# achao2013/deep3dmap

Measured on AMD Instinct MI355X. Metric: rendered Mpix/s fwd+bwd, 100k-tri mesh @512x512, higher is better.
Workload: dtype f32

## Files before the change

deep3dmap_amd/_lib.py:

```python
import ctypes
import os

import torch

from .build import LOAD_PATH as LIB_PATH

_c_f32p = ctypes.c_void_p
_I, _F, _SZ, _L = ctypes.c_int, ctypes.c_float, ctypes.c_size_t, ctypes.c_long
_P = ctypes.c_void_p


class D3MCamera(ctypes.Structure):
    _fields_ = [("mode", _I), ("perspective", _I), ("tan_half_width", _F), ("orig_size", _F),
                ("rot", _P), ("eye_or_t", _P), ("K", _P), ("dist", _P),
                ("rot_batch", _I), ("eye_batch", _I), ("K_batch", _I), ("dist_batch", _I)]


class D3MBasis(ctypes.Structure):
    _fields_ = [("eye", _P), ("at_or_direction", _P), ("up", _P), ("eye_batch", _I), ("at_batch", _I), ("up_batch", _I),
                ("is_look_at", _I)]


class D3MCameraGrad(ctypes.Structure):
    _fields_ = [("eye_or_t", _P), ("at_or_direction", _P), ("up", _P), ("rot", _P), ("K", _P), ("dist", _P)]
# ... 8 lines not shown
    _fields_ = [("intensity_ambient", _P), ("intensity_directional", _P), ("color_ambient", _P), ("color_directional", _P),
                ("direction", _P), ("ia_batch", _I), ("id_batch", _I), ("ca_batch", _I), ("cd_batch", _I), ("dir_batch", _I)]


class D3MMeshTopology(ctypes.Structure):
    _fields_ = ([(n, _P) for n in ("nbr_offsets", "nbr_items", "wings", "wing_offsets", "wing_items", "nbr_chunks",
                                   "nbr_long_rows", "nbr_long_chunk_ptr", "wing_chunks", "wing_long_rows",
                                   "wing_long_chunk_ptr")] +
                [(n, _I) for n in ("num_vertices", "num_edges", "num_wings", "num_nbr_chunks", "num_nbr_long_rows",
                                   "num_wing_chunks", "num_wing_long_rows", "long_row")])


class D3MFitTargets(ctypes.Structure):
    _fields_ = [("rgb_target", _P), ("depth_target", _P), ("alpha_target", _P), ("mask", _P), ("scratch", _P),
                ("loss", _P), ("grad_rgb_map", _P), ("grad_alpha_map", _P), ("grad_depth_map", _P), ("grad_loss", _P),
                ("mask_sum", _P), ("edge_grad", _P), ("edge_dot", _P), ("edge_nz_lo_inv", _P), ("edge_nz_hi1", _P), ("flags", _I)]


class D3MG2SBlock(ctypes.Structure):
    _fields_ = ([("batch_size", _I), ("height", _I), ("width", _I), ("image_size", _I), ("anti_aliasing", _I), ("flip", _I),
                 ("inv_K", _P), ("inv_K_batch", _I), ("K", _P), ("K_batch", _I),
                 ("rot_center_depth", _F), ("depth_min", _F), ("depth_max", _F), ("near", _F), ("far", _F),
                 ("camera", ctypes.POINTER(D3MCamera)), ("view", _P), ("view_components", _I)] +
                [(n, _P) for n in ("rot", "trans", "depth", "albedo", "light_a", "light_b", "light_d", "target", "extra_mask",
                                   "normal", "diffuse_shading", "texture", "recon_depth", "recon_im", "recon_im_mask",
                                   "losses")] +
                [("lam_smooth", _F), ("with_smooth", _I)] +
                [(n, _P) for n in ("screen_vertices", "zbuffer", "scratch",
                                   "grad_recon_im", "grad_l1", "grad_l1_flip", "grad_smooth", "grad_total",
                                   "grad_texture", "grad_tri", "grad_depth_map", "grad_normal", "grad_depth_mesh",
                                   "grad_depth", "grad_albedo", "grad_light_a", "grad_light_b", "grad_light_d", "grad_rot",
# ... 70 lines not shown
    "d3m_face_light": (_I, [_P, _I, _P, _I, _P, _F, _F, _P, _P, _P, _I, _I, _I, _I, _P]),
    "d3m_face_light_backward": (_I, [_P, _I, _P, _I, _P, _P, _F, _F, _P, _P, _P, _I, _I, _I, _I, _P]),
    "d3m_face_light_dev": (_I, [_P, _I, _P, _I, _P, ctypes.POINTER(D3MLight), _I, _I, _I, _I, _P]),
    "d3m_face_light_backward_dev": (_I, [_P, _I, _P, _I, _P, _P, ctypes.POINTER(D3MLight), _I, _I, _I, _I, _P]),
    "d3m_face_light_backward_gather_dev": (_I, [_P, _P, _P, _P, _P, _P, ctypes.POINTER(D3MLight), _I, _I, _I, _P]),
    "d3m_light_params_backward_workspace_bytes": (_SZ, [_I, _I, _I]),
    "d3m_light_params_backward": (_I, [_P, _I, _P, _I, _P, _I, ctypes.POINTER(D3MLight), ctypes.POINTER(D3MLight), _I, _I, _I,
                                       _P, _SZ, _P]),
    "d3m_forward_texture_sampling_lit": (_I, [_P, _P, _I, _P, _I, _P, _P, _P, _P, _I, _I, _I, _I, _I, _F, _P]),
    "d3m_backward_textures_lit_workspace_bytes": (_SZ, [_I, _I, _I, _I]),
    "d3m_render_lit_epilogue": (_I, [_P, _P, _I, _P, _I, _P, _P, _P, _P, _I, _P, _P, _P, _P, _P, _I, _I, _I, _I, _I, _F, _I,
                                     _P, _P]),
    "d3m_render_fit_scratch_floats": (_SZ, [_I, _I]),
    "d3m_render_fit_scratch_clear_range": (_SZ, [_I, _I, ctypes.POINTER(_SZ)]),
    "d3m_fit_finish": (_I, [ctypes.POINTER(D3MFitTargets), _I, _I, _P]),
    "d3m_fit_loss_records": (_I, [_P, _P, _P, _P, ctypes.POINTER(D3MFitTargets), _I, _I, _P]),
    "d3m_backward_textures_lit": (_I, [_P, _P, _I, _P, _I, _P, _P, _P, _P, _P, _P, _P, _P, _I, _I, _I, _I, _I, _F, _P, _SZ,
                                       _P, _P, _P, _I, _P]),
    "d3m_backward_textures_lit_clear_ranges": (_I, [_P, _I, _P, _I, _I, _I, _I, _I, _P, _I, ctypes.POINTER(_P),
                                                    ctypes.POINTER(_SZ)]),
    "d3m_lit_back": (_I, [_P, _I, ctypes.POINTER(D3MCamera), _P, _P, _I, _I, _P, _I, _I, _I, _P, _I, _F, _F, _P, _P, _P, _P]),
    "d3m_lit_back_dev": (_I, [_P, _I, ctypes.POINTER(D3MCamera), _P, _P, _I, _I, _P, _I, _I, _I, _P, _I, ctypes.POINTER(D3MLight),
                              _P]),
    "d3m_lit_front_dev": (_I, [_P, _I, ctypes.POINTER(D3MCamera), ctypes.POINTER(D3MBasis), _P, _I, _I, _P, _I, _I, _I, _P, _I,
                               ctypes.POINTER(D3MLight), ctypes.POINTER(_P), ctypes.POINTER(_SZ), _I, _P]),
    "d3m_lit_front": (_I, [_P, _I, ctypes.POINTER(D3MCamera), ctypes.POINTER(D3MBasis), _P, _I, _I, _P, _I, _I, _I, _P, _I,
                           _F, _F, _P, _P, _P, ctypes.POINTER(_P), ctypes.POINTER(_SZ), _I, _P]),
    "d3m_output_epilogue": (_I, [_P, _P, _P, _P, _I, _P, _P, _P, _P, _P, _I, _I, _I, _P]),
    "d3m_output_epilogue_backward": (_I, [_P, _P, _P, _P, _P, _P, _I, _I, _I, _P]),
    "d3m_output_epilogue_backward_records": (_I, [_P, _P, _P, _P, _P, _P, _P, _P, _P, _P, _P, _I, _I, _I, _P]),
# ... 172 lines not shown
```

deep3dmap_amd/csrc/d3m_edge_grad.h:

```cpp
#pragma once
#include <algorithm>
#include <atomic>
#include <type_traits>
#include "d3m_backward.h"
#include "d3m_face_major.h"
#include "d3m_launch.h"

namespace d3m {

#ifndef D3M_EG_INLINE_MAX
#define D3M_EG_INLINE_MAX 6
#endif
constexpr int EG_INLINE_MAX = D3M_EG_INLINE_MAX;
#ifndef D3M_EG_LINE_WAVES
#define D3M_EG_LINE_WAVES 8
#endif
constexpr int EG_LINE_WAVES = D3M_EG_LINE_WAVES;
constexpr int EG_ITEM_DW = 8;

struct EdgeGradArgs {
    const float4* grad;
    const float2* dot;
    const float* go;
    __device__ __forceinline__ size_t pixel(int axis, size_t view_base, int d0, int d1) const {
// ... 15 lines not shown
    int img_s, img_aa;
    __device__ __forceinline__ bool direct() const { return ga_map != nullptr || ga_img != nullptr; }
    __device__ __forceinline__ float direct_ga(size_t pi) const {
        if (ga_map) return ga_map[pi];
        const size_t plane = (size_t)S * S;
        const int b = (int)(pi / plane), rem = (int)(pi - (size_t)b * plane), y = rem / S, x = rem - y * S;
        const int yo = img_aa ? (S - 1 - y) >> 1 : S - 1 - y, xo = img_aa ? x >> 1 : x;
        return ga_img[((size_t)b * img_s + yo) * img_s + xo] * (img_aa ? 0.25f : 1.0f);
    }
    __device__ __forceinline__ float direct_ga_at(size_t view, int axis, int d0, int d1, size_t pi) const {
        if (ga_map) return ga_map[pi];
        const int y = axis ? d0 : d1, x = axis ? d1 : d0;
        const int yo = img_aa ? (S - 1 - y) >> 1 : S - 1 - y, xo = img_aa ? x >> 1 : x;
        return ga_img[(view * img_s + yo) * img_s + xo] * (img_aa ? 0.25f : 1.0f);
    }
    __device__ __forceinline__ float4 rec_grad(size_t pi) const {
        return direct() ? make_float4(direct_ga(pi), 0.0f, 0.0f, 0.0f) : grad[pi];
    }
    __device__ __forceinline__ float2 rec_dot(size_t pi) const {
        if (!direct()) return dot[pi];
        return make_float2(alpha_map[pi] * direct_ga(pi), __int_as_float(fi_direct[pi]));
    }
    __device__ __forceinline__ int extent_lo(size_t line) const { return nz_lo_inv ? S - nz_lo_inv[line] : 0; }
    __device__ __forceinline__ int extent_hi(size_t line) const { return nz_hi1 ? nz_hi1[line] - 1 : S - 1; }
    int* line_left;
    int* n_left;
};

struct SegRef {
    float alpha, r, g, b;
};

struct Segment {
    int axis, d0, from, to, inward, f0, f1;
// ... 133 lines not shown
__device__ __forceinline__ void visit_pixel_div(float diff, int d1, float d1_cross, float q0, float q1, bool f0, bool f1,
                                                float two_over_is, float eps, float& g0, float& g1) {
    const float t = (float)d1 - d1_cross;
    float dist0 = q0 * t * two_over_is;
    dist0 = (0 < dist0) ? dist0 + eps : dist0 - eps;
    float dist1 = q1 * t * two_over_is;
    dist1 = (0 < dist1) ? dist1 + eps : dist1 - eps;
    const bool skip = diff <= 0;
    g0 -= (skip || !f0) ? 0.0f : diff / dist0;
    g1 -= (skip || !f1) ? 0.0f : diff / dist1;
}

__device__ __forceinline__ SegRef load_ref(const EdgeGradArgs& a, int axis, size_t view_base, int d0, int d1) {
    const size_t idx = view_base + (axis ? (size_t)d0 * a.S + d1 : (size_t)d1 * a.S + d0);
    SegRef r = {0, 0, 0, 0};
    if (a.use_alpha) r.alpha = a.alpha_map[idx];
    if (a.use_rgb) { r.r = a.rgb_map[3 * idx + 0]; r.g = a.rgb_map[3 * idx + 1]; r.b = a.rgb_map[3 * idx + 2]; }
    return r;
}

__device__ __forceinline__ void inline_pixel(const Segment& sg, const SegRef& ref, int fn, const float2 dt, const float4 g,
                                             int d1, bool on, float two_over_is, float eps, float& g0, float& g1) {
    float diff = dt.x;
    diff = __builtin_fmaf(-ref.alpha, g.x, diff);
    diff = __builtin_fmaf(-ref.r, g.y, diff);
    diff = __builtin_fmaf(-ref.g, g.z, diff);
    diff = __builtin_fmaf(-ref.b, g.w, diff);
    if (!on || (sg.inward && __float_as_int(dt.y) != fn)) diff = 0.0f;
    visit_pixel(diff, d1, sg.d1_cross, sg.f0 ? sg.q0 : 1.0f, sg.f1 ? sg.q1 : 1.0f, sg.f0 != 0, sg.f1 != 0, two_over_is, eps,
                g0, g1);
// ... 592 lines not shown
    const size_t view_base = bn * is * is;
    const int x_first = __builtin_amdgcn_readfirstlane(line_first_record(w, line));
    const uint4* xrec = w.xrec + (size_t)x_first;
    const float two_over_is = 2.0f / (float)is;
    const int p_lo = __builtin_amdgcn_readfirstlane(a.extent_lo(line));
    const int p_hi = __builtin_amdgcn_readfirstlane(a.extent_hi(line));
    auto load_record = [&](int ci) {
        uint4 r = make_uint4(0, 0, 0, 0);
        if (ci < n_x) r = xrec[(uint32_t)ci];
        return r;
    };
    float2* s_df = (float2*)s_line;
    float4* s_grd = (float4*)(s_df + is + (is & 1));
    float4* s_val = s_grd + is;
    const float go_sign = a.go_sign();
    for (int p = (int)threadIdx.x; p < is; p += EG_LINE_THREADS) {
        const size_t pi = a.pixel(axis, view_base, d0, p);
        float4 v = make_float4(0, 0, 0, 0);
        if (USE_ALPHA) v.x = a.alpha_map[pi];
        if (USE_RGB) { v.y = a.rgb_map[3 * pi]; v.z = a.rgb_map[3 * pi + 1]; v.w = a.rgb_map[3 * pi + 2]; }
        s_val[p] = v;
    }
    for (int p = p_lo + (int)threadIdx.x; p <= p_hi; p += EG_LINE_THREADS) {
        const size_t pi = a.pixel(axis, view_base, d0, p);
        float4 g;
        float2 d;
        if (!USE_RGB && a.direct()) {
            const float ga = a.direct_ga_at(bn, axis, d0, p, pi);
            g = make_float4(ga, 0.0f, 0.0f, 0.0f);
            d = make_float2(a.alpha_map[pi] * ga, __int_as_float(a.fi_direct[pi]));
        } else {
            g = a.grad[pi];
            d = a.dot[pi];
        }
        g.x *= go_sign; g.y *= go_sign; g.z *= go_sign; g.w *= go_sign;
        s_grd[p] = g;
        s_df[p] = make_float2(0.5f * go_sign * d.x, d.y);
    }
    typedef float v2f __attribute__((ext_vector_type(2)));
    auto diff_of = [](const float4 g, const float2 d, const v2f nref_ar, const v2f nref_gb) {
        v2f p = {d.x, d.x};
        p = __builtin_elementwise_fma(v2f{g.x, g.y}, nref_ar, p);
// ... 754 lines not shown
}

inline size_t edge_grad_workspace_min_bytes(int B, int F, int S) {
    return edge_layout(B, F, S).fixed_bytes + edge_plan_min_bytes(B, F, S);
}
inline size_t edge_grad_workspace_bytes(int B, int F, int S) {
    return edge_layout(B, F, S).fixed_bytes + edge_plan_bytes(B, F, S);
}

struct EdgeRecords {
    const float4* grad;
    const float2* dot;
    const int* nz_lo_inv;
    const int* nz_hi1;
    const float* go;
    const float* ga_img = nullptr;
    int img_aa = 0;
};

inline size_t edge_lines_lds(int S) {
    const size_t pairs = (size_t)(S + (S & 1)) * 8, body = pairs + (size_t)S * 32;
    return std::max(body, pairs + (size_t)(2 * S + 32) * 16);
}

template <class FS>
int run_edge_grad(FS fs, PixelMaps m, float* grad_faces, VertexTarget vt, const VisibilityView* shared_vis,
                  void* shared_plan, size_t shared_plan_bytes, EdgeRecords rec, GradScale gs, int B, float eps, void* ws,
                  size_t ws_bytes, hipStream_t st, int* last_err) {
    const int S = m.S, F = fs.num_faces();
    if (S > 65535 || F > (1 << 25) || (long)B * 2 * S >= (1l << 31)) return 1;
// ... 15 lines not shown
    EdgePlan w;
    if (shared_plan) {
        if (!edge_plan_view(shared_plan, shared_plan_bytes, vis, B, F, S, w)) return 2;
    } else {
        if (!edge_plan_view(p + L.off_plan, ws_bytes - L.fixed_bytes, vis, B, F, S, w)) return 2;
        e = run_edge_plan(fs, m.face_index_map, w, p + L.off_plan, B, S, st);
        if (e != hipSuccess) { *last_err = (int)e; return 3; }
    }
    float4* grad_row = (float4*)(p + L.off_grad_row);
    float2* dot_row = (float2*)(p + L.off_dot_row);
    float2* lane_partial = (float2*)(p + L.off_lane_partial);
    EdgeGradArgs a;
    a.ga_map = a.ga_img = nullptr; a.fi_direct = m.face_index_map; a.img_s = S; a.img_aa = 0;
    const bool direct = !rec.grad && !m.use_rgb && m.use_alpha && !gs.totals &&
                        (rec.ga_img || d3m_env_int("D3M_EG_DIRECT", 1) != 0);
    if (rec.grad) {
        a.grad = rec.grad; a.dot = rec.dot; a.go = rec.go;
        a.nz_lo_inv = rec.nz_lo_inv; a.nz_hi1 = rec.nz_hi1;
    } else if (direct) {
        a.grad = nullptr; a.dot = nullptr; a.go = nullptr; a.nz_lo_inv = a.nz_hi1 = nullptr;
        if (rec.ga_img) { a.ga_img = rec.ga_img; a.img_aa = rec.img_aa; a.img_s = rec.img_aa ? S / 2 : S; }
        else a.ga_map = m.grad_alpha_map;
    } else {
        e = zero_async(p + L.off_nz_lo, L.nz_bytes, st);
        if (e != hipSuccess) { *last_err = (int)e; return 3; }
        LAUNCH("k_pack_maps", k_pack_maps, dim3((S + 31) / 32, (S + 31) / 32, B), dim3(256), st, m.face_index_map,
               m.use_alpha ? m.alpha_map : nullptr, m.use_alpha ? m.grad_alpha_map : nullptr,
               m.use_rgb ? m.rgb_map : nullptr, m.use_rgb ? m.grad_rgb_map : nullptr, grad_row, dot_row,
               (int*)(p + L.off_nz_lo), (int*)(p + L.off_nz_hi), S, gs);
        a.grad = grad_row; a.dot = dot_row; a.go = nullptr;
        a.nz_lo_inv = (const int*)(p + L.off_nz_lo); a.nz_hi1 = (const int*)(p + L.off_nz_hi);
    }
    a.alpha_map = m.alpha_map; a.rgb_map = m.rgb_map;
// ... 48 lines not shown
```

deep3dmap_amd/csrc/d3m_lit.h:

```cpp
#pragma once
#include "d3m_aux.h"
#include "d3m_tail.h"
#include "d3m_face_major.h"

namespace d3m {

struct LitTextures {
    const float* textures;
    const float* light;
    int F, Fp, ts, tex_batch, light_batch, fill_back;
    const float* im;
    int im_H, im_W;
};

__device__ __forceinline__ long lit_texel(const LitTextures& t, int B, int b, int fp, int isc, int* light_row) {
    const int ts3 = t.ts * t.ts * t.ts;
    long vf = (long)b * t.Fp + fp + isc / ts3;
    isc %= ts3;
    if (vf >= (long)B * t.Fp) return -1;
    const int bb = (int)(vf / t.Fp), ff = (int)(vf % t.Fp);
    *light_row = (t.light_batch > 1 ? bb : 0) * t.Fp + ff;
    int fo = ff, idx = isc;
    if (ff >= t.F) {
        fo = ff - t.F;
// ... 413 lines not shown
    }
}

template <int TILE>
__device__ __forceinline__ unsigned tile_row_mask(unsigned long long ball) {
    const int sub = (int)(threadIdx.x & 63) / TILE;
    return (unsigned)(ball >> (sub * TILE)) & (TILE == 32 ? 0xFFFFFFFFu : (1u << (TILE & 31)) - 1u);
}
struct FitRecords {
    float4* grad;
    float2* dot;
    int* nz_lo_inv;
    int* nz_hi1;
    const float* mask_sum;
    float* g_depth;
};

#ifndef D3M_FIT_MINWAVES
#define D3M_FIT_MINWAVES 4
#endif
template <int TILE>
__global__ void __launch_bounds__(256, D3M_FIT_MINWAVES) k_render_lit_fit_records(const float* __restrict__ faces, LitTextures lt,
                                                               const int32_t* __restrict__ face_index_map,
                                                               const float* __restrict__ weight_map,
                                                               const float* __restrict__ depth_map,
                                                               const float* __restrict__ background, int bg_b,
                                                               float* __restrict__ rgb_blended, float* __restrict__ alpha_map,
                                                               float* __restrict__ rgb_out, float* __restrict__ alpha_out,
                                                               float* __restrict__ depth_out,
                                                               int B, int S, float eps, FitTargets fit, FitRecords rec) {
    static_assert(TILE == 32 || TILE == 16, "tile of 32 x 32 or 16 x 16 pixels");
    constexpr int ROWS = 256 / TILE;
    __shared__ float4 s_part[4];
    __shared__ int s_col_lo_inv[TILE], s_col_hi1[TILE];
    if (threadIdx.x < TILE) { s_col_lo_inv[threadIdx.x] = 0; s_col_hi1[threadIdx.x] = 0; }
    __syncthreads();
    const int b = blockIdx.z, x0 = blockIdx.x * TILE, y0 = blockIdx.y * TILE;
    const int tx = threadIdx.x % TILE, ty = threadIdx.x / TILE;
    const float* bg = background + (size_t)(bg_b > 1 ? b : 0) * 3;
    const float inv_pixels = 1.0f / (float)((long)S * S), inv_3den = 1.0f / (3.0f * *rec.mask_sum);
    float t_rgb = 0, t_d = 0, t_m = 0, t_sse = 0;
    auto sgn = [](float x) { return x > 0 ? 1.0f : (x < 0 ? -1.0f : 0.0f); };
    for (int r = ty; r < TILE; r += ROWS) {
        const int yi = y0 + r, xi = x0 + tx;
        bool nz = false;
        if (yi < S && xi < S) {
            const int yo = S - 1 - yi;
            const size_t p = ((size_t)b * S + yi) * S + xi, o = ((size_t)b * S + yo) * S + xi;
            float tg[6];
#pragma unroll
            for (int k = 0; k < 3; k++) tg[k] = fit.rgb_t[(((size_t)b * 3 + k) * S + yo) * S + xi];
            tg[3] = fit.depth_t[o]; tg[4] = fit.alpha_t[o]; tg[5] = fit.mask[o];
            const int fi = face_index_map[p];
            const float depth = depth_map[p];
            float v[3] = {bg[0], bg[1], bg[2]};
            if (fi >= 0) {
                const float weight[3] = {weight_map[3 * p], weight_map[3 * p + 1], weight_map[3 * p + 2]};
                sample_pixel_lit(faces, lt, B, b, fi, weight, depth, eps, v);
            }
            const float alpha = fi >= 0 ? 1.0f : 0.0f;
#pragma unroll
            for (int k = 0; k < 3; k++) rgb_blended[3 * p + k] = v[k];
            alpha_map[p] = alpha;
            if (rgb_out) {
#pragma unroll
                for (int k = 0; k < 3; k++) rgb_out[(((size_t)b * 3 + k) * S + yo) * S + xi] = v[k];
            }
// ... 747 lines not shown
```

deep3dmap_amd/csrc/d3m_raster.hip:

```cpp
#include <hip/hip_runtime.h>
#include <stdint.h>
#include <stdio.h>
#include <string.h>

#include "../../include/d3m_raster.h"
#include "d3m_launch.h"
#include "d3m_aux.h"
#include "d3m_textures.h"
#include "d3m_vertex_colors.h"
#include "d3m_mesh_reg.h"
#include "d3m_morphable.h"
#include "d3m_pose.h"
#include "d3m_mesh.h"
#include "d3m_uv.h"
#include "d3m_backward.h"
#include "d3m_device.h"
#include "d3m_edge_grad.h"
#include "d3m_face_major.h"
#include "d3m_forward.h"
#include "d3m_lit.h"
#include "d3m_g2s.h"
#include "d3m_bid.h"
#include "d3m_front.h"
#include "d3m_light_grad.h"
// ... 426 lines not shown
        num_faces <= 0 || image_size <= 0 || texture_size <= 0)
        return D3M_ERR_INVALID;
    const long n = (long)batch_size * image_size * image_size;
    LAUNCH("k_texture_sampling", k_texture_sampling, dim3(blocks_for(n, 256)), dim3(256), (hipStream_t)stream, faces, textures,
                       face_index_map, weight_map, depth_map, rgb_map, sampling_index_map, sampling_weight_map,
                       batch_size, num_faces, image_size, texture_size, eps);
    return check_launch();
}

static GradScale to_grad_scale(const d3m_fit_targets* unscaled, int image_size) {
    if (!unscaled) return GradScale{nullptr, nullptr, 0.0f, 0, nullptr};
    return GradScale{unscaled->scratch, unscaled->grad_loss, (float)((long)image_size * image_size),
                     unscaled->edge_grad ? 1 : 0, unscaled->mask_sum};
}

D3M_EXPORT size_t d3m_backward_pixel_map_workspace_bytes(int batch_size, int num_faces, int image_size) {
    return edge_grad_workspace_bytes(batch_size, num_faces, image_size);
}

D3M_EXPORT int d3m_backward_pixel_map(const float* faces, const int32_t* face_index_map, const float* rgb_map,
                                      const float* alpha_map, const float* grad_rgb_map, const float* grad_alpha_map,
                                      float* grad_faces, int batch_size, int num_faces, int image_size, float eps,
                                      int return_rgb, int return_alpha, void* workspace, size_t workspace_bytes,
                                      const d3m_vertex_target* vertex_target, void* visibility, void* edge_plan,
                                      size_t edge_plan_size, const d3m_fit_targets* unscaled, d3m_stream_t stream) {
    if (edge_plan && !visibility) return D3M_ERR_INVALID;
    const bool of_image = unscaled && !unscaled->scratch && !unscaled->edge_grad &&
                          (unscaled->flags & D3M_GRAD_OF_OUTPUT_IMAGE) && unscaled->grad_alpha_map;
    if (of_image && (return_rgb || !return_alpha || ((unscaled->flags & D3M_FIT_POOLED) && (image_size & 1))))
        return D3M_ERR_INVALID;
// ... 5 lines not shown
    if (int rc = to_vertex_target(vertex_target, num_faces, vt)) return rc;
    const bool records = unscaled && unscaled->edge_grad;
    if (records && !(unscaled->edge_dot && unscaled->edge_nz_lo_inv && unscaled->edge_nz_hi1)) return D3M_ERR_INVALID;
    if (return_rgb && (!rgb_map || (!grad_rgb_map && !records))) return D3M_ERR_INVALID;
    if (return_alpha && (!alpha_map || (!grad_alpha_map && !records && !of_image))) return D3M_ERR_INVALID;
    if (!return_rgb && !return_alpha) return D3M_OK;
    DenseFaces fs{faces, num_faces};
    PixelMaps m{face_index_map, rgb_map, alpha_map, grad_rgb_map, grad_alpha_map, image_size, return_rgb != 0,
                return_alpha != 0};
    VisibilityView vis;
    if (visibility) vis = visibility_view(visibility, (long)batch_size * num_faces);
    EdgeRecords rec{nullptr, nullptr, nullptr, nullptr, nullptr};
    if (records)
        rec = EdgeRecords{(const float4*)unscaled->edge_grad, (const float2*)unscaled->edge_dot, unscaled->edge_nz_lo_inv,
                          unscaled->edge_nz_hi1, unscaled->grad_loss};
    if (of_image) {
        rec.ga_img = unscaled->grad_alpha_map;
        rec.img_aa = (unscaled->flags & D3M_FIT_POOLED) ? 1 : 0;
    }
    return run_edge_grad(fs, m, grad_faces, vt, visibility ? &vis : nullptr, edge_plan, edge_plan_size, rec,
                         to_grad_scale(of_image ? nullptr : unscaled, image_size), batch_size, eps, workspace, workspace_bytes,
                         (hipStream_t)stream, &g_last_hip_error);
}

D3M_EXPORT size_t d3m_backward_pixel_map_workspace_min_bytes(int batch_size, int num_faces, int image_size) {
    return edge_grad_workspace_min_bytes(batch_size, num_faces, image_size);
}

D3M_EXPORT size_t d3m_edge_plan_bytes(int batch_size, int num_faces, int image_size) {
    if (batch_size <= 0 || num_faces <= 0 || image_size <= 0) return 0;
// ... 770 lines not shown
                                                const float* weight_map, const float* depth_map, float* rgb_map,
                                                int batch_size, int num_tri, int fill_back, int image_size,
                                                int texture_size, float eps, d3m_stream_t stream) {
    if (!faces || !face_index_map || !weight_map || !depth_map || !rgb_map || batch_size <= 0 || image_size <= 0)
        return D3M_ERR_INVALID;
    LitTextures lt;
    int rc = make_lit(lt, textures, textures_batch, light, light_batch, num_tri, texture_size, fill_back, batch_size);
    if (rc) return rc;
    const long n = (long)batch_size * image_size * image_size;
    LAUNCH("k_texture_sampling_lit", k_texture_sampling_lit, dim3(blocks_for(n, 256)), dim3(256), (hipStream_t)stream, faces, lt,
           face_index_map, weight_map, depth_map, rgb_map, batch_size, image_size, eps);
    return check_launch();
}

struct FitScratch {
    size_t off_partials, off_group_sums, off_tickets, ticket_words, floats;
};
static const long FIT_TILE16_MAX_PIXELS = 4l << 20;
static int fit_tile(int B, int S) { return (long)B * S * S <= FIT_TILE16_MAX_PIXELS ? 16 : 32; }
static FitScratch fit_scratch_layout(int B, int S) {
    const size_t per_pixels = blocks_for((long)B * S * S, 256);
    const size_t tiles32 = (size_t)B * ((S + 31) / 32) * ((S + 31) / 32), tiles16 = (size_t)B * ((S + 15) / 16) * ((S + 15) / 16);
    const size_t tiles = tiles32 > tiles16 ? tiles32 : tiles16;
    const size_t P = per_pixels > tiles ? per_pixels : tiles;
    const size_t G = std::max((size_t)B, (per_pixels + 255) / 256);
    FitScratch L;
    L.off_partials = 8;
    L.off_group_sums = 8 + 4 * P;
    L.off_tickets = L.off_group_sums + 4 * G;
    L.ticket_words = 4;
    L.floats = L.off_tickets + L.ticket_words;
    return L;
}
D3M_EXPORT size_t d3m_render_fit_scratch_floats(int batch_size, int image_size) {
    if (batch_size <= 0 || image_size <= 0) return 0;
    return fit_scratch_layout(batch_size, image_size).floats;
}
D3M_EXPORT size_t d3m_render_fit_scratch_clear_range(int batch_size, int image_size, size_t* offset_floats) {
    if (batch_size <= 0 || image_size <= 0) return 0;
    const FitScratch L = fit_scratch_layout(batch_size, image_size);
    if (offset_floats) *offset_floats = L.off_tickets;
    return L.ticket_words;
}

static int to_fit_targets(const d3m_fit_targets* fit, FitTargets& ft) {
    ft = FitTargets{nullptr, nullptr, nullptr, nullptr, nullptr, nullptr, nullptr, nullptr};
    if (!fit) return D3M_OK;
    if (!fit->rgb_target || !fit->depth_target || !fit->alpha_target || !fit->mask || !fit->scratch || !fit->loss)
        return D3M_ERR_INVALID;
    const bool any = fit->grad_rgb_map || fit->grad_alpha_map || fit->grad_depth_map;
    if (any && !fit->edge_grad && !(fit->grad_rgb_map && fit->grad_alpha_map && fit->grad_depth_map)) return D3M_ERR_INVALID;
// ... 38 lines not shown
    if (rc) return rc;
    FitTargets ft;
    const int s = anti_aliasing ? image_size / 2 : image_size;
    if ((rc = to_fit_targets(fit, ft))) return rc;
    const long n = (long)batch_size * s * s;
    hipStream_t st = (hipStream_t)stream;
    const int threads = 256;
    if (fit && (rc = clear_fit_tickets(fit, batch_size, image_size, st))) return rc;
    if (fit && fit->edge_grad) {
        if (!fit->edge_dot || !fit->edge_nz_lo_inv || !fit->edge_nz_hi1 || !fit->mask_sum || !fit->grad_depth_map)
            return D3M_ERR_INVALID;
        const dim3 tiles((image_size + 31) / 32, (image_size + 31) / 32, batch_size);
        const dim3 tiles16((image_size + 15) / 16, (image_size + 15) / 16, batch_size);
        FitRecords rec{(float4*)fit->edge_grad, (float2*)fit->edge_dot, fit->edge_nz_lo_inv, fit->edge_nz_hi1, fit->mask_sum,
                       fit->grad_depth_map};
        if (anti_aliasing)
            LAUNCH("k_render_lit_fit_records", k_render_lit_fit_records_pooled, tiles, dim3(256), st, faces, lt,
                   face_index_map, weight_map, depth_map, background, background_batch, rgb_blended, alpha_map, rgb_out,
                   alpha_out, depth_out, batch_size, image_size, eps, ft, rec);
        else if (fit_tile(batch_size, image_size) == 16)
            LAUNCH("k_render_lit_fit_records", k_render_lit_fit_records<16>, tiles16, dim3(256), st, faces, lt, face_index_map,
                   weight_map, depth_map, background, background_batch, rgb_blended, alpha_map, rgb_out, alpha_out,
                   depth_out, batch_size, image_size, eps, ft, rec);
        else
            LAUNCH("k_render_lit_fit_records", k_render_lit_fit_records<32>, tiles, dim3(256), st, faces, lt, face_index_map,
                   weight_map, depth_map, background, background_batch, rgb_blended, alpha_map, rgb_out, alpha_out,
                   depth_out, batch_size, image_size, eps, ft, rec);
        if (!(fit->flags & D3M_FIT_FINISH_DEFERRED)) {
            const FitFin fin = fit_fin_of_tiles(fit, batch_size, image_size);
            LAUNCH("k_fit_finish", k_fit_finish, dim3(fin.n_groups), dim3(256), st, fin);
// ... 14 lines not shown
D3M_EXPORT int d3m_fit_finish(const d3m_fit_targets* fit, int batch_size, int image_size, d3m_stream_t stream) {
    if (!fit || !fit->scratch || !fit->loss || !fit->edge_grad || batch_size <= 0 || image_size <= 0) return D3M_ERR_INVALID;
    const FitFin fin = fit_fin_of_tiles(fit, batch_size, image_size);
    LAUNCH("k_fit_finish", k_fit_finish, dim3(fin.n_groups), dim3(256), (hipStream_t)stream, fin);
    return check_launch();
}

D3M_EXPORT int d3m_fit_loss_records(const float* rgb, const float* depth, const float* alpha, const int32_t* face_index_map,
                                    const d3m_fit_targets* fit, int batch_size, int image_size, d3m_stream_t stream) {
    if (!rgb || !depth || !alpha || !face_index_map || !fit || batch_size <= 0 || image_size <= 0) return D3M_ERR_INVALID;
    if (!fit->edge_grad || !fit->edge_dot || !fit->edge_nz_lo_inv || !fit->edge_nz_hi1 || !fit->mask_sum || !fit->grad_depth_map)
        return D3M_ERR_INVALID;
    FitTargets ft;
    if (int rc = to_fit_targets(fit, ft)) return rc;
    if (fit->flags & (D3M_FIT_FINISH_DEFERRED | D3M_FIT_POOLED)) return D3M_ERR_INVALID;
    hipStream_t st = (hipStream_t)stream;
    if (int rc = clear_fit_tickets(fit, batch_size, image_size, st)) return rc;
    FitRecords rec{(float4*)fit->edge_grad, (float2*)fit->edge_dot, fit->edge_nz_lo_inv, fit->edge_nz_hi1, fit->mask_sum,
                   fit->grad_depth_map};
    if (fit_tile(batch_size, image_size) == 16)
        LAUNCH("k_fit_loss_records", k_fit_loss_records<16>, dim3((image_size + 15) / 16, (image_size + 15) / 16, batch_size),
               dim3(256), st, rgb, depth, alpha, face_index_map, batch_size, image_size, ft, rec);
    else
        LAUNCH("k_fit_loss_records", k_fit_loss_records<32>, dim3((image_size + 31) / 32, (image_size + 31) / 32, batch_size),
               dim3(256), st, rgb, depth, alpha, face_index_map, batch_size, image_size, ft, rec);
    const FitFin fin = fit_fin_of_tiles(fit, batch_size, image_size);
    LAUNCH("k_fit_finish", k_fit_finish, dim3(fin.n_groups), dim3(256), st, fin);
    return check_launch();
}

struct LitWorkspace {
    float* gview;
    int* flags;
    unsigned* view_mask;
    size_t mask_bytes;
    int* n_large;
    size_t total;
};
static LitWorkspace lit_workspace(void* ws, int B, int num_tri, int fill_back, int texture_size) {
    const size_t ts3 = (size_t)texture_size * texture_size * texture_size;
    const size_t nf = (size_t)B * num_tri * (fill_back ? 2 : 1);
    char* p = (char*)ws;
// ... 966 lines not shown
```

deep3dmap_amd/neural_renderer/rasterize.py:

```python
import collections
import ctypes
import dataclasses
import os
from typing import Any, NamedTuple, Optional

import torch
import torch.nn as nn

from .. import _lib
from . import rasterize_ops as ops
from ._util import const_tensor, deterministic as _deterministic, f32c
from .row_gather import vertex_adjacency

DEFAULT_IMAGE_SIZE = 256
DEFAULT_ANTI_ALIASING = True
DEFAULT_NEAR = 0.1
DEFAULT_FAR = 100
DEFAULT_EPS = 1e-4
DEFAULT_BACKGROUND_COLOR = (0, 0, 0)


def _background_tensor(background_color, device):
    if background_color is None:
        background_color = DEFAULT_BACKGROUND_COLOR
    if torch.is_tensor(background_color):
        t = background_color.to(device=device, dtype=torch.float32)
# ... 292 lines not shown

def _image_grad_struct(g_img, pooled):
    return _lib.D3MFitTargets(grad_alpha_map=_lib.ptr(g_img), flags=_lib.GRAD_OF_OUTPUT_IMAGE | (_lib.FIT_POOLED if pooled else 0))


class _FitState(NamedTuple):
    rgb_t: torch.Tensor
    depth_t: torch.Tensor
    alpha_t: torch.Tensor
    mask: torch.Tensor
    scratch: list
    loss: torch.Tensor
    mask_sum: Optional[torch.Tensor]
    pooled: bool
    records: Optional[_Records]

    def struct(self, k, lo, hi, grad_loss=None, flags=0):
        rec = self.records.fields(lo, hi) if self.records is not None else {}
        if self.records is not None and self.pooled:
            flags = int(flags) | _lib.FIT_POOLED
        return _lib.D3MFitTargets(
            rgb_target=_lib.ptr(self.rgb_t[lo:hi]), depth_target=_lib.ptr(self.depth_t[lo:hi]),
            alpha_target=_lib.ptr(self.alpha_t[lo:hi]), mask=_lib.ptr(self.mask[lo:hi]), scratch=_lib.ptr(self.scratch[k]),
            loss=_lib.ptr(self.loss[k:k + 1]), grad_loss=_lib.ptr(grad_loss), mask_sum=_lib.ptr(self.mask_sum), **rec,
            flags=int(flags))


def _front_clears(clears):
    assert len(clears) <= _lib.FRONT_RANGES
    n = max(1, len(clears))
    return (ctypes.c_void_p * n)(*[c[0] for c in clears]), (ctypes.c_size_t * n)(*[c[1] for c in clears]), len(clears)


def _check_deterministic(det):
    if _deterministic() != det:
        raise RuntimeError("the deterministic mode (D3M_DETERMINISTIC, d3m_set_deterministic) was %s for this render node's "
                           "forward pass and is %s for its backward pass: the deterministic() block must enclose backward "
                           "as well as forward" % (("on", "off") if det else ("off", "on")))


# ... 262 lines not shown
        serial = G == 1 and (det or manual or _serial_branches(B, Ft, S))
        mains = [cur] + [_side_stream(dev, k) for k in range(1, G)]
        auxs = [_side_stream(dev, G + k, serial) for k in range(G)]
        own_extents = False
        if objective is not None:
            records = None
            if need_grad:
                extents = None
                if serial and plan is not None:
                    each = ctypes.c_size_t(0)
                    off = int(L.d3m_edge_plan_extents_offset(B, Fp, S, ctypes.byref(each)))
                    extents = tuple(plan[0][off + j * each.value: off + j * each.value + B * 2 * S * 4].view(torch.int32)
                                    .view(B, 2, S) for j in range(2))
                own_extents = extents is None
                records = _pixel_records(B, S, dev, grad_depth=True, extents=extents)
            fit_state = _FitState(rgb_t, depth_t, alpha_t, mask, scratch, loss_g, mask_sum, bool(anti_aliasing), records)
        st = _LitState(S=S, eps=float(eps), aa=bool(anti_aliasing), ra=bool(return_alpha), rd=bool(return_depth),
                       fill_back=bool(fill_back), light=(float(ia), float(idr), ca, cd, direction) if dlight is None else None,
                       Bl=Bl, groups=groups, need_grad=need_grad, need_geom=need_geom, need_tex=need_tex,
                       need_vert=need_vert, gathered=need_tex or need_vert or any(need_lp) or any(need_cp), det=det,
                       serial=serial,
                       plan_open=bool(plan is not None and defer_plan_join and G == 1),
                       camera=camera, cam_keep=cam_keep, grad_sink=grad_sink,
                       fit=None if hinted else fit_state, hint=fit_state if hinted else None,
                       hint_mask_sum_given=hinted and mask_sum_given, dlight=dlight, need_lp=need_lp,
                       need_mesh=need_mesh, need_cp=need_cp, adjacency=adjacency)
        clears, pre = [], None
        flags_fwd = flags_plan = flags_fit = 0
        ws0 = ops._workspace("fwd", L.d3m_forward_workspace_bytes(groups[0][1] - groups[0][0], Fp, S), dev)
        if G == 1:
            nb = int(L.d3m_forward_clear_bytes(B, Ft, int(bool(fill_back)), S, ws0.numel()))
# ... 640 lines not shown
```

include/d3m_raster.h:

```cpp
#ifndef D3M_RASTER_H
#define D3M_RASTER_H

#include <stddef.h>
#include <stdint.h>

#ifdef __cplusplus
extern "C" {
#endif

typedef void* d3m_stream_t;

enum {
    D3M_OK = 0,
    D3M_ERR_INVALID = 1,
    D3M_ERR_WORKSPACE = 2,
    D3M_ERR_LAUNCH = 3
};

enum { D3M_CAMERA_NONE = 0, D3M_CAMERA_LOOK_AT = 1, D3M_CAMERA_LOOK = 2, D3M_CAMERA_PROJECTION = 3 };

const char* d3m_version(void);
int d3m_last_hip_error(void);
int d3m_zero_ranges(void* const* ptrs, const size_t* bytes, int count, d3m_stream_t stream);
#define D3M_PRECLEARED 1
// ... 237 lines not shown
    const float* depth_target;
    const float* alpha_target;
    const float* mask;
    float* scratch;
    float* loss;
    float* grad_rgb_map;
    float* grad_alpha_map;
    float* grad_depth_map;
    const float* grad_loss;
    const float* mask_sum;
    void* edge_grad;
    void* edge_dot;
    int* edge_nz_lo_inv;
    int* edge_nz_hi1;
    int flags;
};
#define D3M_FIT_FINISH_DEFERRED 2
#define D3M_FIT_POOLED 4
int d3m_fit_finish(const d3m_fit_targets* fit, int batch_size, int image_size, d3m_stream_t stream);
size_t d3m_render_fit_scratch_floats(int batch_size, int image_size);
size_t d3m_render_fit_scratch_clear_range(int batch_size, int image_size, size_t* offset_floats);
int d3m_fit_loss_records(const float* rgb, const float* depth, const float* alpha, const int32_t* face_index_map,
                         const d3m_fit_targets* fit, int batch_size, int image_size, d3m_stream_t stream);
int d3m_render_lit_epilogue(const float* faces, const float* textures, int textures_batch, const float* light,
                            int light_batch, const int32_t* face_index_map, const float* weight_map,
                            const float* depth_map, const float* background, int background_batch,
                            float* rgb_blended, float* alpha_map, float* rgb_out, float* alpha_out, float* depth_out,
                            int batch_size, int num_tri, int fill_back, int image_size, int texture_size, float eps,
                            int anti_aliasing, const d3m_fit_targets* fit, d3m_stream_t stream);
size_t d3m_backward_textures_lit_workspace_bytes(int batch_size, int num_tri, int fill_back, int texture_size);
int d3m_backward_textures_lit(const float* faces, const float* textures, int textures_batch, const float* light,
                              int light_batch, const int32_t* face_index_map, const float* weight_map,
                              const float* depth_map, const float* grad_rgb_map, float* grad_textures, float* grad_light,
                              const float* grad_depth_map, float* grad_faces, int batch_size, int num_tri, int fill_back,
                              int image_size, int texture_size, float eps, void* workspace, size_t workspace_bytes,
                              const d3m_vertex_target* vertex_target, void* visibility,
// ... 173 lines not shown
```

Measured before the change: 5837.

## Skip empty fit tiles using cached per-tile target void summary

Adds a cached per-16x16-tile summary of fit targets (zero alpha and mask, finite depth and rgb). The fused lit-epilogue fit kernel uses it to mark tiles that are void in the target and uncovered by any face. For those tiles it writes background outputs and zero loss partials, then exits early. The edge-gradient kernel treats such pixels as fixed background with zero gradient instead of reading per-pixel records, saving memory traffic on empty screen regions. The risks are extra branches per pixel access in the edge kernel, a target summary that can go stale if targets change in place (the cache is keyed on the tensors), and a new global tile-size override.

```diff
diff --git a/deep3dmap_amd/_lib.py b/deep3dmap_amd/_lib.py
--- a/deep3dmap_amd/_lib.py
+++ b/deep3dmap_amd/_lib.py
@@ -46,7 +46,8 @@
 class D3MFitTargets(ctypes.Structure):
     _fields_ = [("rgb_target", _P), ("depth_target", _P), ("alpha_target", _P), ("mask", _P), ("scratch", _P),
                 ("loss", _P), ("grad_rgb_map", _P), ("grad_alpha_map", _P), ("grad_depth_map", _P), ("grad_loss", _P),
-                ("mask_sum", _P), ("edge_grad", _P), ("edge_dot", _P), ("edge_nz_lo_inv", _P), ("edge_nz_hi1", _P), ("flags", _I)]
+                ("mask_sum", _P), ("edge_grad", _P), ("edge_dot", _P), ("edge_nz_lo_inv", _P), ("edge_nz_hi1", _P), ("flags", _I),
+                ("tile_void", _P)]
 
 
 class D3MG2SBlock(ctypes.Structure):
@@ -147,6 +148,10 @@
     "d3m_render_fit_scratch_floats": (_SZ, [_I, _I]),
     "d3m_render_fit_scratch_clear_range": (_SZ, [_I, _I, ctypes.POINTER(_SZ)]),
     "d3m_fit_finish": (_I, [ctypes.POINTER(D3MFitTargets), _I, _I, _P]),
+    "d3m_render_fit_scratch_tile_void_offset": (_SZ, [_I, _I]),
+    "d3m_fit_target_summary": (_I, [_P, _P, _P, _P, _P, _I, _I, _P]),
+    "d3m_set_fit_tile_form": (_I, [_I]),
+    "d3m_get_fit_tile_form": (_I, []),
     "d3m_fit_loss_records": (_I, [_P, _P, _P, _P, ctypes.POINTER(D3MFitTargets), _I, _I, _P]),
     "d3m_backward_textures_lit": (_I, [_P, _P, _I, _P, _I, _P, _P, _P, _P, _P, _P, _P, _P, _I, _I, _I, _I, _I, _F, _P, _SZ,
                                        _P, _P, _P, _I, _P]),
diff --git a/deep3dmap_amd/csrc/d3m_edge_grad.h b/deep3dmap_amd/csrc/d3m_edge_grad.h
--- a/deep3dmap_amd/csrc/d3m_edge_grad.h
+++ b/deep3dmap_amd/csrc/d3m_edge_grad.h
@@ -53,10 +53,29 @@
         const int yo = img_aa ? (S - 1 - y) >> 1 : S - 1 - y, xo = img_aa ? x >> 1 : x;
         return ga_img[(view * img_s + yo) * img_s + xo] * (img_aa ? 0.25f : 1.0f);
     }
+    const unsigned char* tile_void;
+    const float* void_bg;
+    int tile_shift, tiles_x, tiles_view;
+    __device__ __forceinline__ bool void_at(size_t view, int axis, int d0, int d1) const {
+        if (!tile_void) return false;
+        const int y = axis ? d0 : d1, x = axis ? d1 : d0;
+        return tile_void[view * tiles_view + (size_t)(y >> tile_shift) * tiles_x + (x >> tile_shift)] != 0;
+    }
+    __device__ __forceinline__ bool void_pixel(size_t pi) const {
+        if (!tile_void) return false;
+        const size_t plane = (size_t)S * S, b = pi / plane;
+        const int rem = (int)(pi - b * plane), y = rem / S;
+        return void_at(b, 1, y, rem - y * S);
+    }
+    __device__ __forceinline__ float4 void_value(size_t view) const {
+        return make_float4(0.0f, void_bg[4 * view], void_bg[4 * view + 1], void_bg[4 * view + 2]);
+    }
     __device__ __forceinline__ float4 rec_grad(size_t pi) const {
+        if (void_pixel(pi)) return make_float4(0.0f, 0.0f, 0.0f, 0.0f);
         return direct() ? make_float4(direct_ga(pi), 0.0f, 0.0f, 0.0f) : grad[pi];
     }
     __device__ __forceinline__ float2 rec_dot(size_t pi) const {
+        if (void_pixel(pi)) return make_float2(0.0f, __int_as_float(-1));
         if (!direct()) return dot[pi];
         return make_float2(alpha_map[pi] * direct_ga(pi), __int_as_float(fi_direct[pi]));
     }
@@ -220,6 +239,11 @@
 __device__ __forceinline__ SegRef load_ref(const EdgeGradArgs& a, int axis, size_t view_base, int d0, int d1) {
     const size_t idx = view_base + (axis ? (size_t)d0 * a.S + d1 : (size_t)d1 * a.S + d0);
     SegRef r = {0, 0, 0, 0};
+    if (a.void_pixel(idx)) {
+        const float4 v = a.void_value(idx / ((size_t)a.S * a.S));
+        r.r = v.y; r.g = v.z; r.b = v.w;
+        return r;
+    }
     if (a.use_alpha) r.alpha = a.alpha_map[idx];
     if (a.use_rgb) { r.r = a.rgb_map[3 * idx + 0]; r.g = a.rgb_map[3 * idx + 1]; r.b = a.rgb_map[3 * idx + 2]; }
     return r;
@@ -842,18 +866,26 @@
     float4* s_grd = (float4*)(s_df + is + (is & 1));
     float4* s_val = s_grd + is;
     const float go_sign = a.go_sign();
+    constexpr bool VOID_TILES = USE_RGB && USE_ALPHA;
     for (int p = (int)threadIdx.x; p < is; p += EG_LINE_THREADS) {
         const size_t pi = a.pixel(axis, view_base, d0, p);
         float4 v = make_float4(0, 0, 0, 0);
-        if (USE_ALPHA) v.x = a.alpha_map[pi];
-        if (USE_RGB) { v.y = a.rgb_map[3 * pi]; v.z = a.rgb_map[3 * pi + 1]; v.w = a.rgb_map[3 * pi + 2]; }
+        if (VOID_TILES && a.void_at(bn, axis, d0, p)) {
+            v = a.void_value(bn);
+        } else {
+            if (USE_ALPHA) v.x = a.alpha_map[pi];
+            if (USE_RGB) { v.y = a.rgb_map[3 * pi]; v.z = a.rgb_map[3 * pi + 1]; v.w = a.rgb_map[3 * pi + 2]; }
+        }
         s_val[p] = v;
     }
     for (int p = p_lo + (int)threadIdx.x; p <= p_hi; p += EG_LINE_THREADS) {
         const size_t pi = a.pixel(axis, view_base, d0, p);
         float4 g;
         float2 d;
-        if (!USE_RGB && a.direct()) {
+        if (VOID_TILES && a.void_at(bn, axis, d0, p)) {
+            g = make_float4(0.0f, 0.0f, 0.0f, 0.0f);
+            d = make_float2(0.0f, __int_as_float(-1));
+        } else if (!USE_RGB && a.direct()) {
             const float ga = a.direct_ga_at(bn, axis, d0, p, pi);
             g = make_float4(ga, 0.0f, 0.0f, 0.0f);
             d = make_float2(a.alpha_map[pi] * ga, __int_as_float(a.fi_direct[pi]));
@@ -1638,6 +1670,9 @@
     const int* nz_lo_inv;
     const int* nz_hi1;
     const float* go;
+    const unsigned char* tile_void = nullptr;
+    const float* void_bg = nullptr;
+    int tile = 0;
     const float* ga_img = nullptr;
     int img_aa = 0;
 };
@@ -1683,9 +1718,16 @@
     a.ga_map = a.ga_img = nullptr; a.fi_direct = m.face_index_map; a.img_s = S; a.img_aa = 0;
     const bool direct = !rec.grad && !m.use_rgb && m.use_alpha && !gs.totals &&
                         (rec.ga_img || d3m_env_int("D3M_EG_DIRECT", 1) != 0);
+    a.tile_void = nullptr; a.void_bg = nullptr; a.tile_shift = 0; a.tiles_x = a.tiles_view = 0;
     if (rec.grad) {
         a.grad = rec.grad; a.dot = rec.dot; a.go = rec.go;
         a.nz_lo_inv = rec.nz_lo_inv; a.nz_hi1 = rec.nz_hi1;
+        if (rec.tile_void) {
+            if (!(m.use_rgb && m.use_alpha) || !rec.void_bg || (rec.tile != 16 && rec.tile != 32)) return 1;
+            a.tile_void = rec.tile_void; a.void_bg = rec.void_bg;
+            a.tile_shift = rec.tile == 32 ? 5 : 4;
+            a.tiles_x = (S + rec.tile - 1) / rec.tile; a.tiles_view = a.tiles_x * a.tiles_x;
+        }
     } else if (direct) {
         a.grad = nullptr; a.dot = nullptr; a.go = nullptr; a.nz_lo_inv = a.nz_hi1 = nullptr;
         if (rec.ga_img) { a.ga_img = rec.ga_img; a.img_aa = rec.img_aa; a.img_s = rec.img_aa ? S / 2 : S; }
diff --git a/deep3dmap_amd/csrc/d3m_lit.h b/deep3dmap_amd/csrc/d3m_lit.h
--- a/deep3dmap_amd/csrc/d3m_lit.h
+++ b/deep3dmap_amd/csrc/d3m_lit.h
@@ -451,7 +451,25 @@
     int* nz_hi1;
     const float* mask_sum;
     float* g_depth;
+    const unsigned char* target_void = nullptr;
+    unsigned char* tile_void = nullptr;
+    float* void_bg = nullptr;
 };
+
+__global__ void __launch_bounds__(256) k_fit_target_summary(const float* __restrict__ rgb_t, const float* __restrict__ depth_t,
+                                                           const float* __restrict__ alpha_t, const float* __restrict__ mask,
+                                                           unsigned char* __restrict__ target_void, int B, int S) {
+    const int b = blockIdx.z, xo = blockIdx.x * 16 + (threadIdx.x & 15), yo = blockIdx.y * 16 + (threadIdx.x >> 4);
+    bool live = false;
+    if (xo < S && yo < S) {
+        const size_t o = ((size_t)b * S + yo) * S + xo;
+        live = !(alpha_t[o] == 0.0f) || !(mask[o] == 0.0f) || !isfinite(depth_t[o]);
+#pragma unroll
+        for (int k = 0; k < 3; k++) live = live || !isfinite(rgb_t[(((size_t)b * 3 + k) * S + yo) * S + xo]);
+    }
+    const int any = __syncthreads_or(live ? 1 : 0);
+    if (threadIdx.x == 0) target_void[((size_t)b * gridDim.y + blockIdx.y) * gridDim.x + blockIdx.x] = any ? 0 : 1;
+}
 
 #ifndef D3M_FIT_MINWAVES
 #define D3M_FIT_MINWAVES 4
@@ -478,16 +496,52 @@
     const float inv_pixels = 1.0f / (float)((long)S * S), inv_3den = 1.0f / (3.0f * *rec.mask_sum);
     float t_rgb = 0, t_d = 0, t_m = 0, t_sse = 0;
     auto sgn = [](float x) { return x > 0 ? 1.0f : (x < 0 ? -1.0f : 0.0f); };
+    bool t_void = false;
+    if (rec.target_void) {
+        const int n16 = (S + 15) >> 4, xe = min(x0 + TILE, S) - 1, yo_lo = S - min(y0 + TILE, S), yo_hi = S - 1 - y0;
+        t_void = isfinite(bg[0]) && isfinite(bg[1]) && isfinite(bg[2]) && isfinite(inv_3den);
+        for (int j = yo_lo >> 4; j <= yo_hi >> 4; j++)
+            for (int i = x0 >> 4; i <= xe >> 4; i++) t_void = t_void && rec.target_void[((size_t)b * n16 + j) * n16 + i] != 0;
+        if (blockIdx.x == 0 && blockIdx.y == 0 && threadIdx.x < 3) rec.void_bg[4 * b + threadIdx.x] = bg[threadIdx.x];
+        const size_t tile = ((size_t)blockIdx.z * gridDim.y + blockIdx.y) * gridDim.x + blockIdx.x;
+        bool covered = false;
+        if (t_void) {
+            for (int r = ty; r < TILE; r += ROWS)
+                if (y0 + r < S && x0 + tx < S) covered = covered || face_index_map[((size_t)b * S + y0 + r) * S + x0 + tx] >= 0;
+            covered = __syncthreads_or(covered ? 1 : 0) != 0;
+        }
+        if (threadIdx.x == 0) rec.tile_void[tile] = (t_void && !covered) ? 1 : 0;
+        if (t_void && !covered) {
+            if (threadIdx.x == 0) reinterpret_cast<float4*>(fit.partials)[tile] = make_float4(0, 0, 0, 0);
+            if (rgb_out || alpha_out || depth_out) {
+                for (int r = ty; r < TILE; r += ROWS) {
+                    const int yi = y0 + r, xi = x0 + tx;
+                    if (yi >= S || xi >= S) continue;
+                    const int yo = S - 1 - yi;
+                    const size_t o = ((size_t)b * S + yo) * S + xi;
+                    if (rgb_out) {
+#pragma unroll
+                        for (int k = 0; k < 3; k++) rgb_out[(((size_t)b * 3 + k) * S + yo) * S + xi] = bg[k];
+                    }
+                    if (alpha_out) alpha_out[o] = 0.0f;
+                    if (depth_out) depth_out[o] = depth_map[((size_t)b * S + yi) * S + xi];
+                }
+            }
+            return;
+        }
+    }
     for (int r = ty; r < TILE; r += ROWS) {
         const int yi = y0 + r, xi = x0 + tx;
         bool nz = false;
         if (yi < S && xi < S) {
             const int yo = S - 1 - yi;
             const size_t p = ((size_t)b * S + yi) * S + xi, o = ((size_t)b * S + yo) * S + xi;
-            float tg[6];
-#pragma unroll
-            for (int k = 0; k < 3; k++) tg[k] = fit.rgb_t[(((size_t)b * 3 + k) * S + yo) * S + xi];
-            tg[3] = fit.depth_t[o]; tg[4] = fit.alpha_t[o]; tg[5] = fit.mask[o];
+            float tg[6] = {0, 0, 0, 0, 0, 0};
+            if (!t_void) {
+#pragma unroll
+                for (int k = 0; k < 3; k++) tg[k] = fit.rgb_t[(((size_t)b * 3 + k) * S + yo) * S + xi];
+                tg[3] = fit.depth_t[o]; tg[4] = fit.alpha_t[o]; tg[5] = fit.mask[o];
+            }
             const int fi = face_index_map[p];
             const float depth = depth_map[p];
             float v[3] = {bg[0], bg[1], bg[2]};
diff --git a/deep3dmap_amd/csrc/d3m_raster.hip b/deep3dmap_amd/csrc/d3m_raster.hip
--- a/deep3dmap_amd/csrc/d3m_raster.hip
+++ b/deep3dmap_amd/csrc/d3m_raster.hip
@@ -464,6 +464,8 @@
                      unscaled->edge_grad ? 1 : 0, unscaled->mask_sum};
 }
 
+static void fit_void_records(const d3m_fit_targets* unscaled, int B, int S, EdgeRecords& rec);
+
 D3M_EXPORT size_t d3m_backward_pixel_map_workspace_bytes(int batch_size, int num_faces, int image_size) {
     return edge_grad_workspace_bytes(batch_size, num_faces, image_size);
 }
@@ -499,6 +501,7 @@
     if (records)
         rec = EdgeRecords{(const float4*)unscaled->edge_grad, (const float2*)unscaled->edge_dot, unscaled->edge_nz_lo_inv,
                           unscaled->edge_nz_hi1, unscaled->grad_loss};
+    if (records) fit_void_records(unscaled, batch_size, image_size, rec);
     if (of_image) {
         rec.ga_img = unscaled->grad_alpha_map;
         rec.img_aa = (unscaled->flags & D3M_FIT_POOLED) ? 1 : 0;
@@ -1299,10 +1302,21 @@
 }
 
 struct FitScratch {
-    size_t off_partials, off_group_sums, off_tickets, ticket_words, floats;
+    size_t off_partials, off_group_sums, off_tickets, ticket_words, off_void_bg, off_tile_void, floats;
 };
 static const long FIT_TILE16_MAX_PIXELS = 4l << 20;
-static int fit_tile(int B, int S) { return (long)B * S * S <= FIT_TILE16_MAX_PIXELS ? 16 : 32; }
+static std::atomic<int> g_fit_tile_form{-1};
+D3M_EXPORT int d3m_set_fit_tile_form(int form) {
+    if (form < -1 || form > 1) return D3M_ERR_INVALID;
+    g_fit_tile_form.store(form);
+    return D3M_OK;
+}
+D3M_EXPORT int d3m_get_fit_tile_form(void) { return g_fit_tile_form.load(); }
+static int fit_tile(int B, int S) {
+    const int form = g_fit_tile_form.load();
+    if (form >= 0) return form ? 32 : 16;
+    return (long)B * S * S <= FIT_TILE16_MAX_PIXELS ? 16 : 32;
+}
 static FitScratch fit_scratch_layout(int B, int S) {
     const size_t per_pixels = blocks_for((long)B * S * S, 256);
     const size_t tiles32 = (size_t)B * ((S + 31) / 32) * ((S + 31) / 32), tiles16 = (size_t)B * ((S + 15) / 16) * ((S + 15) / 16);
@@ -1314,12 +1328,28 @@
     L.off_group_sums = 8 + 4 * P;
     L.off_tickets = L.off_group_sums + 4 * G;
     L.ticket_words = 4;
-    L.floats = L.off_tickets + L.ticket_words;
+    L.off_void_bg = L.off_tickets + L.ticket_words;
+    L.off_tile_void = L.off_void_bg + 4 * (size_t)B;
+    L.floats = L.off_tile_void + (tiles + 3) / 4;
     return L;
+}
+static bool fit_void_tiles(const d3m_fit_targets* fit) {
+    return fit && fit->tile_void && fit->edge_grad && fit->scratch && !(fit->flags & D3M_FIT_POOLED);
+}
+static void fit_void_records(const d3m_fit_targets* unscaled, int B, int S, EdgeRecords& rec) {
+    if (!fit_void_tiles(unscaled)) return;
+    const FitScratch L = fit_scratch_layout(B, S);
+    rec.tile_void = (const unsigned char*)(unscaled->scratch + L.off_tile_void);
+    rec.void_bg = unscaled->scratch + L.off_void_bg;
+    rec.tile = fit_tile(B, S);
 }
 D3M_EXPORT size_t d3m_render_fit_scratch_floats(int batch_size, int image_size) {
     if (batch_size <= 0 || image_size <= 0) return 0;
     return fit_scratch_layout(batch_size, image_size).floats;
+}
+D3M_EXPORT size_t d3m_render_fit_scratch_tile_void_offset(int batch_size, int image_size) {
+    if (batch_size <= 0 || image_size <= 0) return 0;
+    return fit_scratch_layout(batch_size, image_size).off_tile_void;
 }
 D3M_EXPORT size_t d3m_render_fit_scratch_clear_range(int batch_size, int image_size, size_t* offset_floats) {
     if (batch_size <= 0 || image_size <= 0) return 0;
@@ -1388,6 +1418,12 @@
         const dim3 tiles16((image_size + 15) / 16, (image_size + 15) / 16, batch_size);
         FitRecords rec{(float4*)fit->edge_grad, (float2*)fit->edge_dot, fit->edge_nz_lo_inv, fit->edge_nz_hi1, fit->mask_sum,
                        fit->grad_depth_map};
+        if (fit_void_tiles(fit)) {
+            const FitScratch L = fit_scratch_layout(batch_size, image_size);
+            rec.target_void = fit->tile_void;
+            rec.void_bg = fit->scratch + L.off_void_bg;
+            rec.tile_void = (unsigned char*)(fit->scratch + L.off_tile_void);
+        }
         if (anti_aliasing)
             LAUNCH("k_render_lit_fit_records", k_render_lit_fit_records_pooled, tiles, dim3(256), st, faces, lt,
                    face_index_map, weight_map, depth_map, background, background_batch, rgb_blended, alpha_map, rgb_out,
@@ -1432,6 +1468,7 @@
     FitTargets ft;
     if (int rc = to_fit_targets(fit, ft)) return rc;
     if (fit->flags & (D3M_FIT_FINISH_DEFERRED | D3M_FIT_POOLED)) return D3M_ERR_INVALID;
+    if (fit->tile_void) return D3M_ERR_INVALID;
     hipStream_t st = (hipStream_t)stream;
     if (int rc = clear_fit_tickets(fit, batch_size, image_size, st)) return rc;
     FitRecords rec{(float4*)fit->edge_grad, (float2*)fit->edge_dot, fit->edge_nz_lo_inv, fit->edge_nz_hi1, fit->mask_sum,
@@ -1444,6 +1481,17 @@
                dim3(256), st, rgb, depth, alpha, face_index_map, batch_size, image_size, ft, rec);
     const FitFin fin = fit_fin_of_tiles(fit, batch_size, image_size);
     LAUNCH("k_fit_finish", k_fit_finish, dim3(fin.n_groups), dim3(256), st, fin);
+    return check_launch();
+}
+
+D3M_EXPORT int d3m_fit_target_summary(const float* rgb_target, const float* depth_target, const float* alpha_target,
+                                      const float* mask, unsigned char* tile_void, int batch_size, int image_size,
+                                      d3m_stream_t stream) {
+    if (!rgb_target || !depth_target || !alpha_target || !mask || !tile_void || batch_size <= 0 || image_size <= 0)
+        return D3M_ERR_INVALID;
+    const int n16 = (image_size + 15) / 16;
+    LAUNCH("k_fit_target_summary", k_fit_target_summary, dim3(n16, n16, batch_size), dim3(256), (hipStream_t)stream,
+           rgb_target, depth_target, alpha_target, mask, tile_void, batch_size, image_size);
     return check_launch();
 }
 
diff --git a/deep3dmap_amd/neural_renderer/rasterize.py b/deep3dmap_amd/neural_renderer/rasterize.py
--- a/deep3dmap_amd/neural_renderer/rasterize.py
+++ b/deep3dmap_amd/neural_renderer/rasterize.py
@@ -10,6 +10,7 @@
 from .. import _lib
 from . import rasterize_ops as ops
 from ._util import const_tensor, deterministic as _deterministic, f32c
+from .built_cache import BuiltCache, tensor_key
 from .row_gather import vertex_adjacency
 
 DEFAULT_IMAGE_SIZE = 256
@@ -332,6 +333,7 @@
     mask_sum: Optional[torch.Tensor]
     pooled: bool
     records: Optional[_Records]
+    tile_void: Optional[torch.Tensor] = None
 
     def struct(self, k, lo, hi, grad_loss=None, flags=0):
         rec = self.records.fields(lo, hi) if self.records is not None else {}
@@ -341,7 +343,43 @@
             rgb_target=_lib.ptr(self.rgb_t[lo:hi]), depth_target=_lib.ptr(self.depth_t[lo:hi]),
             alpha_target=_lib.ptr(self.alpha_t[lo:hi]), mask=_lib.ptr(self.mask[lo:hi]), scratch=_lib.ptr(self.scratch[k]),
             loss=_lib.ptr(self.loss[k:k + 1]), grad_loss=_lib.ptr(grad_loss), mask_sum=_lib.ptr(self.mask_sum), **rec,
-            flags=int(flags))
+            flags=int(flags), tile_void=_lib.ptr(None if self.tile_void is None else self.tile_void[lo:hi]))
+
+
+class _TargetVoidCache(BuiltCache):
+    what = "the fit targets' void-tile summary"
+
+
+_target_void_cache = _TargetVoidCache(size=2)
+
+
+def fit_void_tiles_enabled():
+    return os.environ.get("D3M_FIT_VOID_TILES", "1") != "0"
+
+
+def _build_target_void(rgb_t, depth_t, alpha_t, mask):
+    B, S = mask.shape[0], mask.shape[-1]
+    n16 = (S + 15) // 16
+    out = torch.empty(B, n16, n16, dtype=torch.uint8, device=mask.device)
+    _lib.check(_lib.lib().d3m_fit_target_summary(_lib.ptr(rgb_t), _lib.ptr(depth_t), _lib.ptr(alpha_t), _lib.ptr(mask),
+                                                 _lib.ptr(out), B, S, _lib.stream_ptr()), "d3m_fit_target_summary")
+    return out
+
+
+def target_void_summary(rgb_t, depth_t, alpha_t, mask, build=_build_target_void, capturing=None):
+    if not fit_void_tiles_enabled():
+        return None
+    targets = (rgb_t, depth_t, alpha_t, mask)
+    key = tuple(tensor_key(t) for t in targets)
+    if capturing is None:
+        capturing = torch.cuda.is_available() and torch.cuda.is_current_stream_capturing()
+    if capturing and key not in _target_void_cache:
+        return None
+    return _target_void_cache.get(key, lambda: build(*targets), holders=targets)
+
+
+def invalidate_target_void_summaries():
+    _target_void_cache.clear()
 
 
 def _front_clears(clears):
@@ -634,7 +672,11 @@
                                     .view(B, 2, S) for j in range(2))
                 own_extents = extents is None
                 records = _pixel_records(B, S, dev, grad_depth=True, extents=extents)
-            fit_state = _FitState(rgb_t, depth_t, alpha_t, mask, scratch, loss_g, mask_sum, bool(anti_aliasing), records)
+            tile_void = None
+            if records is not None and not anti_aliasing and not hinted:
+                tile_void = target_void_summary(rgb_t, depth_t, alpha_t, mask)
+            fit_state = _FitState(rgb_t, depth_t, alpha_t, mask, scratch, loss_g, mask_sum, bool(anti_aliasing), records,
+                                  tile_void)
         st = _LitState(S=S, eps=float(eps), aa=bool(anti_aliasing), ra=bool(return_alpha), rd=bool(return_depth),
                        fill_back=bool(fill_back), light=(float(ia), float(idr), ca, cd, direction) if dlight is None else None,
                        Bl=Bl, groups=groups, need_grad=need_grad, need_geom=need_geom, need_tex=need_tex,
diff --git a/include/d3m_raster.h b/include/d3m_raster.h
--- a/include/d3m_raster.h
+++ b/include/d3m_raster.h
@@ -275,12 +275,18 @@
     int* edge_nz_lo_inv;
     int* edge_nz_hi1;
     int flags;
+    const unsigned char* tile_void;
 };
 #define D3M_FIT_FINISH_DEFERRED 2
 #define D3M_FIT_POOLED 4
+int d3m_fit_target_summary(const float* rgb_target, const float* depth_target, const float* alpha_target, const float* mask,
+                           unsigned char* tile_void, int batch_size, int image_size, d3m_stream_t stream);
+int d3m_set_fit_tile_form(int form);
+int d3m_get_fit_tile_form(void);
 int d3m_fit_finish(const d3m_fit_targets* fit, int batch_size, int image_size, d3m_stream_t stream);
 size_t d3m_render_fit_scratch_floats(int batch_size, int image_size);
 size_t d3m_render_fit_scratch_clear_range(int batch_size, int image_size, size_t* offset_floats);
+size_t d3m_render_fit_scratch_tile_void_offset(int batch_size, int image_size);
 int d3m_fit_loss_records(const float* rgb, const float* depth, const float* alpha, const int32_t* face_index_map,
                          const d3m_fit_targets* fit, int batch_size, int image_size, d3m_stream_t stream);
 int d3m_render_lit_epilogue(const float* faces, const float* textures, int textures_batch, const float* light,
diff --git a/tools_dev/void_share.py b/tools_dev/void_share.py
--- /dev/null
+++ b/tools_dev/void_share.py
@@ -0,0 +1,29 @@
+import json, sys, os
+sys.path.insert(0, os.path.dirname(os.path.dirname(os.path.abspath(__file__))))
+import numpy as np, torch
+from deep3dmap_amd import synthetic
+from deep3dmap_amd.multiview import MultiViewFit
+out = {}
+for name, mesh_n, S, views in (("headline", 225, 512, 32), ("8-view shard", 225, 512, 8), ("config 5", 709, 1024, 8)):
+    v, tri = synthetic.grid_mesh(mesh_n)
+    tex = synthetic.random_textures(tri.shape[0], 2)
+    fit = MultiViewFit(v, tri, tex, synthetic.camera_ring(views), image_size=S, anti_aliasing=False, rank=0, world_size=1,
+                       device="cuda:0", objective_in_renderer=True)
+    fit.set_targets_from(synthetic.perturb(v))
+    fit.keep_images = True
+    fit.step()
+    torch.cuda.synchronize()
+    rgb_t, depth_t, alpha_t = (t.cpu().numpy() for t in fit.targets[:3])
+    alpha = fit.images[2].cpu().numpy()
+    ok = (alpha_t == 0) & np.isfinite(depth_t) & np.isfinite(rgb_t).all(1)
+    r = {"covered_pixels": float((alpha > 0).mean()), "target_live_pixels": float((alpha_t != 0).mean())}
+    for T in (16, 32):
+        n = S // T
+        tv = ok.reshape(views, n, T, n, T).all((2, 4))
+        cov = (alpha > 0).reshape(views, n, T, n, T).any((2, 4))
+        r[f"tile{T}"] = {"target_void": float(tv.mean()), "void": float((tv & ~cov).mean())}
+    out[name] = r
+    del fit
+os.makedirs("dev_out", exist_ok=True)
+json.dump(out, open("dev_out/void_tiles_share.json", "w"), indent=1)
+print(json.dumps(out))
```

Result: faster. 5986 (median of 6 runs) (+2.6%).
